# tsinghua-fib-lab/PIML

Measured on AMD Instinct MI355X. Metric: agent-pair force evals/sec + simulated steps/sec, 4096-agent GC scene, higher is better.
Workload: dtype f32

## Files before the change

piml_amd/csrc/encoder_bwd5.hip:

```cpp
#include "common.hpp"
#include "encoder.hpp"
#include "x3.hpp"

namespace piml {

typedef short f5_s16x4 __attribute__((ext_vector_type(4)));
typedef __attribute__((address_space(3))) f5_s16x4 f5_lds_s16x4;

constexpr int F5_THREADS = 512;
constexpr int F5_IMG = 3 * 128 * 64;
constexpr int F5_M = 0;
constexpr int F5_H = F5_M + 2 * F5_IMG;
constexpr int F5_TROW = 36;
constexpr int F5_TBYTES = 128 * F5_TROW * 4;
constexpr int F5_T = F5_H + 2 * F5_IMG;
constexpr int F5_XS = F5_T + 2 * F5_TBYTES;
constexpr int F5_MK = F5_XS + 3 * 1024;
constexpr int F5_W1 = F5_MK + 2 * 512;
constexpr int F5_GXP = F5_W1 + 4096;
#ifndef PIML_F5_PHASED
#define PIML_F5_PHASED 1
#endif
#ifndef PIML_F5_REQ_EARLY
#define PIML_F5_REQ_EARLY 0
#endif
#ifndef PIML_F5_GX_MFMA
#define PIML_F5_GX_MFMA 1
#endif
#ifndef PIML_F5_DW1_MFMA
#define PIML_F5_DW1_MFMA 0
#endif
static_assert(!PIML_F5_GX_MFMA || PIML_F5_PHASED, "the g_x products ride in the phased schedule");
static_assert(!PIML_F5_DW1_MFMA || PIML_F5_GX_MFMA, "the dW1 products need the zero region the g_x products freed");
constexpr int F5_GXP_BYTES = PIML_F5_GX_MFMA ? 4 * 32 * 16 * 4 : 4096;
constexpr int F5_TAB = F5_GXP + 2 * F5_GXP_BYTES;
constexpr int F5_KMAX = 16;
constexpr int F5_LDS_BYTES = F5_TAB + F5_KMAX * 2 * 16 * 4;
constexpr int F5_LDS_LAUNCH = F5_LDS_BYTES;
static_assert(F5_LDS_LAUNCH <= 160 * 1024, "fits the CU");
constexpr int F5_PART1 = EH * EH + 1024 + 2 * EH;

struct F5Args {
    EncArgs A;
    int nA[2];
    DecSlotSums D;
};

#ifndef PIML_F5_DEC_AT
#define PIML_F5_DEC_AT 1
#endif

template <int C>
__device__ __forceinline__ float f5_row_shl(float v) {
    return __int_as_float(__builtin_amdgcn_mov_dpp(__float_as_int(v), 0x100 + C, 0xf, 0xf, false));
}
template <int C>
__device__ __forceinline__ void f5_chains_add(float4& s, const float4 v) {
    if constexpr (C < 16) {
        slot_chains_add(s, make_float4(f5_row_shl<C>(v.x), f5_row_shl<C>(v.y), f5_row_shl<C>(v.z), f5_row_shl<C>(v.w)));
        f5_chains_add<C + 1>(s, v);
    }
}
__device__ __forceinline__ void f5_dec_sums(const DecSlotSums& D, int wg, int nwg, int t, int nthr) {
    const int total = D.nsets * D.lanes, per = (total + nwg - 1) / nwg;
    const int e1 = min(wg * per + per, total), half = nthr >> 4;
    for (int e = wg * per + (t >> 4); e < e1; e += 2 * half) {
        const bool two = e + half < e1;
        const int ea = e, eb = two ? e + half : e;
        const int sa = ea >= D.lanes ? 1 : 0, sb = eb >= D.lanes ? 1 : 0;
        const float4* const p[2] = {reinterpret_cast<const float4*>(sa ? D.parts[1] : D.parts[0]),
                                    reinterpret_cast<const float4*>(sb ? D.parts[1] : D.parts[0])};
        const int j[2] = {ea - sa * D.lanes, eb - sb * D.lanes};
        float4 s[2];
        slot_chains<2>(p, D.slots, D.lanes, j, t & 15, s);
        const float4 va = s[0], vb = s[1];
        f5_chains_add<1>(s[0], va);
        f5_chains_add<1>(s[1], vb);
        if ((t & 15) == 0) {
            slot_sum_store(reinterpret_cast<float4*>(sa ? D.grads[1] : D.grads[0]) + j[0], s[0], D.accumulate != 0);
            if (two) slot_sum_store(reinterpret_cast<float4*>(sb ? D.grads[1] : D.grads[0]) + j[1], s[1], D.accumulate != 0);
        }
    }
}

#ifdef PIML_F5_STAMPS
__device__ unsigned long long g_f5_stamps[256 * 8 * 16];
#define F5_STAMP(i)                                                        \
    do {                                                                   \
        __builtin_amdgcn_sched_barrier(0);                                 \
        {                                                                  \
            const unsigned long long t_ = __builtin_amdgcn_s_memtime();    \
            st[i] += t_ - tprev;                                           \
            tprev = t_;                                                    \
        }                                                                  \
        __builtin_amdgcn_sched_barrier(0);                                 \
    } while (0)
#else
#define F5_STAMP(i)
#endif

#define F5_BARRIER() asm volatile("s_waitcnt lgkmcnt(0)\n\ts_barrier" ::: "memory")

__device__ __forceinline__ float f5_relu(float x) { return __int_as_float(max(__float_as_int(x), 0)); }
__device__ __forceinline__ constexpr int f5_rho(int r) { return (r & 3) + 8 * (r >> 2); }

#ifndef PIML_F5_SKIP
#define PIML_F5_SKIP 0
#endif

#define F5_SLOT(MF, FILL)                        \
    do {                                         \
        MF;                                      \
        __builtin_amdgcn_sched_barrier(0);       \
        FILL;                                    \
        __builtin_amdgcn_sched_barrier(0);       \
    } while (0)

template <bool GX, int INC>
__global__ __launch_bounds__(F5_THREADS) void enc_bwd_sums2_kernel(F5Args F) {
    extern __shared__ __align__(16) unsigned char smem[];
    const int tid = threadIdx.x, lane = tid & 63;
    const int wv = __builtin_amdgcn_readfirstlane(tid >> 6);
    const int crew = wv >> 2, w = wv & 3;
    const int ctid = tid & 255;
    const int n = lane & 31, h = lane >> 5;
    int bx = (int)blockIdx.x, b = 0;
    if (bx >= F.nA[0]) { b = 1; bx -= F.nA[0]; }
    const piml_encoder_branch J = b ? F.A.br[1] : F.A.br[0];
    const int nwg = F.nA[b];
    const unsigned R = (unsigned)J.rows;
    const unsigned IN = __builtin_amdgcn_readfirstlane((unsigned)J.in_dim), K = __builtin_amdgcn_readfirstlane((unsigned)J.k);
    const unsigned kmagic = __builtin_amdgcn_readfirstlane((unsigned)((0x100000000ull + K - 1) / K));
    const int ntiles = (int)((R + 31) >> 5);
    const int nit = bx < ntiles ? (ntiles - bx + nwg - 1) / nwg : 0;
    float* P = J.partials + (size_t)bx * F5_PART1;
    constexpr int NS = INC == 6 ? 3 : 4;

    auto rsrc = [&](const void* base, unsigned bytes) {
        return __builtin_amdgcn_make_buffer_rsrc(const_cast<void*>(base), 0, (int)bytes, 0x00020000);
    };
    constexpr unsigned kOut = 0x80000000u;
    const __amdgpu_buffer_rsrc_t rs_gp = rsrc(J.g_pooled, (R / K) * EH * 4);
    const __amdgpu_buffer_rsrc_t rs_x = rsrc(J.x, R * IN * 4);
    const __amdgpu_buffer_rsrc_t rs_mk = rsrc(J.relu_mask, (unsigned)ntiles * 1024);
    const __amdgpu_buffer_rsrc_t rs_gx = rsrc(J.g_x, GX ? R * IN * 4 : 0u);
    auto ld1 = [&](const __amdgpu_buffer_rsrc_t& rs, unsigned voff, unsigned soff) {
        return (unsigned)__builtin_amdgcn_raw_buffer_load_b32(rs, (int)voff, (int)soff, 0);
    };

#ifdef PIML_F5_STAMPS
    unsigned long long st[16], tprev = __builtin_amdgcn_s_memtime();
#pragma unroll
    for (int i = 0; i < 16; ++i) st[i] = 0;
#endif

    {
        float4* z = reinterpret_cast<float4*>(smem + F5_T);
        constexpr int NZ = (F5_W1 - F5_T) / 16;
#pragma unroll
        for (int i = 0; i < (NZ + F5_THREADS - 1) / F5_THREADS; ++i)
            if (i * F5_THREADS + tid < NZ) z[i * F5_THREADS + tid] = make_float4(0.f, 0.f, 0.f, 0.f);
#pragma unroll
        for (int i = 0; i < 2 * F5_GXP_BYTES / 16 / F5_THREADS; ++i) reinterpret_cast<float4*>(smem + F5_GXP)[i * F5_THREADS + tid] = make_float4(0.f, 0.f, 0.f, 0.f);
        if ((unsigned)tid < K * 32u) {
            const unsigned rem = (unsigned)tid >> 5, hh = ((unsigned)tid >> 4) & 1u, r = (unsigned)tid & 15u;
            reinterpret_cast<unsigned*>(smem + F5_TAB)[tid] = ((rem + 4u * hh + (unsigned)f5_rho((int)r)) / K) * (EH * 4);
        }
        if (tid < 256 && PIML_F5_GX_MFMA) {
            reinterpret_cast<float4*>(smem + F5_W1)[tid] = make_float4(0.f, 0.f, 0.f, 0.f);
        } else if (tid < 256) {
            const float* W1r = J.packed + PACK_FWD + 32768;
            if (INC == 6) {
                const float* src = W1r + (tid >> 1) * 8 + 3 * (tid & 1);
                reinterpret_cast<float4*>(smem + F5_W1)[tid] = make_float4(src[0], src[1], src[2], 0.f);
            } else {
                reinterpret_cast<float4*>(smem + F5_W1)[tid] = reinterpret_cast<const float4*>(W1r)[tid];
            }
        }
    }

    if (crew == 0) {
        u32x4 wh[8], wm[8], wl[8];
        {
            const u32x4* imgB = reinterpret_cast<const u32x4*>(J.packed + PACK_F32 + 3 * X3_IMG) + lane;
#pragma unroll
            for (int kb = 0; kb < 8; ++kb) {
                const int fb = w * 8 + kb;
                wh[kb] = imgB[(fb * 2) * 64];
                wm[kb] = imgB[(fb * 2 + 1) * 64];
                wl[kb] = imgB[X3_HM / 4 + fb * 64];
            }
        }
        const float* W1rows = J.packed + PACK_FWD + 32768;
        float w1v[NS];
#pragma unroll
        for (int s = 0; s < NS; ++s) w1v[s] = W1rows[(32 * w + n) * 8 + 2 * s + h];
        const float b1v = J.b1[32 * w + n];

        const int fw = 32 * w + n;
        const int swz_w = (fw >> 1) & 7;
        const int mw_off = F5_M + fw * 64;
        int mr[2];
        {
            const int g16 = lane >> 4, q = (lane >> 2) & 3, pp = lane & 3, hh = g16 >> 1;
            const int chunk = 4 * (g16 & 1) + pp;
#pragma unroll
            for (int half2 = 0; half2 < 2; ++half2)
                mr[half2] = F5_M + (8 * half2 + 4 * hh + q) * 64 + ((chunk ^ (4 * half2 + 2 * hh + (q >> 1))) * 8);
        }
        const int bp = 16 * (w & 1) + (n & 3) + 4 * (n >> 3);
        const int mk_off = F5_MK + ((4 * h + 32 * ((n >> 2) & 1)) * 2 + (w >> 1)) * 4;
        const int t_off = F5_T + fw * (F5_TROW * 4) + (4 * h) * 4;
        const int h_off = F5_H + ((w * 2) * 3 * 64 + lane) * 16;
        const unsigned gbase = (unsigned)(32 * w + n) * 4u;

        float g2[16];
        unsigned m2 = 0, mkv = 0;
        float xa[NS];
        auto req_g = [&](int tile) {
            const unsigned t32 = __builtin_amdgcn_readfirstlane((unsigned)tile * 32u);
            const unsigned a0 = __builtin_amdgcn_readfirstlane(__umulhi(t32, kmagic)), rem = t32 - a0 * K;
            const bool live = tile < ntiles;
            const unsigned gb = live ? gbase + a0 * (EH * 4) : kOut;
            const uint4* tab = reinterpret_cast<const uint4*>(smem + F5_TAB + (rem * 32u + 16u * (unsigned)h) * 4u);
#pragma unroll
            for (int i = 0; i < 4; ++i) {
                const uint4 o = tab[i];
                g2[4 * i + 0] = __uint_as_float(ld1(rs_gp, gb + o.x, 0u));
                g2[4 * i + 1] = __uint_as_float(ld1(rs_gp, gb + o.y, 0u));
                g2[4 * i + 2] = __uint_as_float(ld1(rs_gp, gb + o.z, 0u));
                g2[4 * i + 3] = __uint_as_float(ld1(rs_gp, gb + o.w, 0u));
            }
            m2 = ld1(rs_mk, live ? (unsigned)tile * 1024u + (128u + 2u * (unsigned)lane + (unsigned)(w >> 1)) * 4u : kOut, 0u);
        };
        auto req_x = [&](int tile) {
            const unsigned row = (unsigned)tile * 32u + (unsigned)n;
            const bool valid = (tile < ntiles) & (row < R);
#pragma unroll
            for (int s = 0; s < NS; ++s) {
                const unsigned cx = 2u * s + h;
                xa[s] = __uint_as_float(ld1(rs_x, (valid & (cx < IN)) ? (row * IN + cx) * 4u : kOut, 0u));
            }
            mkv = ld1(rs_mk, tile < ntiles ? (unsigned)tile * 1024u + (unsigned)(ctid & 127) * 4u : kOut, 0u);
        };
        float g2n[16];
        unsigned m2n = 0, mkvn = 0;
        float xan[NS];
        uint4 tabv;
        auto req_step = [&](int i, int tile) {
            const unsigned t32 = __builtin_amdgcn_readfirstlane((unsigned)tile * 32u);
            const unsigned a0 = __builtin_amdgcn_readfirstlane(__umulhi(t32, kmagic)), rem = t32 - a0 * K;
            const bool live = tile < ntiles;
            const uint4* tab = reinterpret_cast<const uint4*>(smem + F5_TAB + (rem * 32u + 16u * (unsigned)h) * 4u);
            if (i == 0) { tabv = tab[0]; return; }
            if (i <= 4) {
                const unsigned gb = live ? gbase + a0 * (EH * 4) : kOut;
                const uint4 o = tabv;
                if (i < 4) tabv = tab[i];
                g2n[4 * i - 4] = __uint_as_float(ld1(rs_gp, gb + o.x, 0u));
                g2n[4 * i - 3] = __uint_as_float(ld1(rs_gp, gb + o.y, 0u));
                g2n[4 * i - 2] = __uint_as_float(ld1(rs_gp, gb + o.z, 0u));
                g2n[4 * i - 1] = __uint_as_float(ld1(rs_gp, gb + o.w, 0u));
                return;
            }
            m2n = ld1(rs_mk, live ? (unsigned)tile * 1024u + (128u + 2u * (unsigned)lane + (unsigned)(w >> 1)) * 4u : kOut, 0u);
            const unsigned row = (unsigned)tile * 32u + (unsigned)n;
            const bool valid = live & (row < R);
#pragma unroll
            for (int s = 0; s < NS; ++s) {
                const unsigned cx = 2u * s + h;
                xan[s] = __uint_as_float(ld1(rs_x, (valid & (cx < IN)) ? (row * IN + cx) * 4u : kOut, 0u));
            }
            mkvn = ld1(rs_mk, live ? (unsigned)tile * 1024u + (unsigned)(ctid & 127) * 4u : kOut, 0u);
        };
        auto req_take = [&]() {
#pragma unroll
            for (int r = 0; r < 16; ++r) g2[r] = g2n[r];
#pragma unroll
            for (int s = 0; s < NS; ++s) xa[s] = xan[s];
            m2 = m2n; mkv = mkvn;
        };
        float db1 = 0.f, db2 = 0.f;
        unsigned phi[4], pmid[4], plo[4];
        float sp_ra = 0.f, sp_rb = 0.f;
        auto split_a = [&](float a_, float b_, unsigned& hi) {
            hi = bf16_pair(a_, b_);
            sp_ra = a_ - __uint_as_float(hi << 16);
            sp_rb = b_ - __uint_as_float(hi & 0xffff0000u);
        };
        auto split_b = [&](unsigned& mid, unsigned& lo) {
            mid = bf16_pair(sp_ra, sp_rb);
            lo = bf16_pair(sp_ra - __uint_as_float(mid << 16), sp_rb - __uint_as_float(mid & 0xffff0000u));
        };
        auto g2_step = [&](int j, int pm) {
            const int s = j >> 3, q = j & 7;
            if (q < 2) {
                const unsigned m2w = m2 >> (16 * (w & 1));
#pragma unroll
                for (int r = 8 * s + 4 * q; r < 8 * s + 4 * q + 4; ++r) {
                    const int t = __builtin_amdgcn_sbfe(m2w, r, 1);
                    g2[r] = __uint_as_float(__float_as_uint(g2[r]) & (unsigned)t);
                    db2 += g2[r];
                }
            } else if (q < 6) {
                const int d = q - 2;
                split_a(g2[8 * s + 2 * d], g2[8 * s + 2 * d + 1], phi[d]);
                split_b(pmid[d], plo[d]);
            } else {
                const int g = 2 * s + (q - 6), d = 2 * (g & 1);
                unsigned char* dst = smem + mw_off + pm * F5_IMG + (((2 * g + h) ^ swz_w) * 8);
                *reinterpret_cast<uint2*>(dst) = make_uint2(phi[d], phi[d + 1]);
                *reinterpret_cast<uint2*>(dst + 8192) = make_uint2(pmid[d], pmid[d + 1]);
                *reinterpret_cast<uint2*>(dst + 16384) = make_uint2(plo[d], plo[d + 1]);
            }
        };
        f32x16 hacc;
        auto h1_mma = [&]() {
#pragma unroll
            for (int r = 0; r < 16; ++r) hacc[r] = b1v;
#pragma unroll
            for (int s = 0; s < NS; ++s) hacc = mfma32(xa[s], w1v[s], hacc);
        };
        auto h1_step = [&](int j, int pm) {
            const int s = j / 5, q = j % 5;
            if (q < 4) {
                split_a(f5_relu(hacc[8 * s + 2 * q]), f5_relu(hacc[8 * s + 2 * q + 1]), phi[q]);
                split_b(pmid[q], plo[q]);
            } else {
                u32x4* dst = reinterpret_cast<u32x4*>(smem + h_off + pm * F5_IMG + (s * 3 * 64) * 16);
                dst[0] = (u32x4){phi[0], phi[1], phi[2], phi[3]};
                dst[64] = (u32x4){pmid[0], pmid[1], pmid[2], pmid[3]};
                dst[128] = (u32x4){plo[0], plo[1], plo[2], plo[3]};
            }
        };
        auto stage = [&](int xslot, int pm) {
            if (w < NS) reinterpret_cast<float*>(smem + F5_XS + xslot * 1024)[n * 8 + 2 * w + h] = w == 0 ? xa[0] : (w == 1 ? xa[1] : (w == 2 ? xa[2] : xa[NS - 1]));
            if (ctid < 128) reinterpret_cast<unsigned*>(smem + F5_MK + pm * 512)[ctid] = mkv;
        };
        auto load_b = [&](u32x4 (&o)[3], int kb, int pm) {
#pragma unroll
            for (int p = 0; p < 3; ++p) {
                const f5_s16x4 lo4 = __builtin_amdgcn_ds_read_tr16_b64_v4i16((f5_lds_s16x4*)(smem + mr[0] + pm * F5_IMG + kb * 1024 + p * 8192));
                const f5_s16x4 hi4 = __builtin_amdgcn_ds_read_tr16_b64_v4i16((f5_lds_s16x4*)(smem + mr[1] + pm * F5_IMG + kb * 1024 + p * 8192));
                const uint2 x = __builtin_bit_cast(uint2, lo4), y = __builtin_bit_cast(uint2, hi4);
                o[p] = (u32x4){x.x, x.y, y.x, y.y};
            }
        };

        F5_BARRIER();
        req_g(bx);
        req_x(bx);
#pragma unroll
        for (int j = 0; j < 16; ++j) g2_step(j, 0);
        h1_mma();
#pragma unroll
        for (int j = 0; j < 10; ++j) h1_step(j, 0);
        stage(0, 0);
        req_g(bx + nwg);
        req_x(bx + nwg);
        F5_STAMP(15);
        F5_BARRIER();

        for (int it = 0; it < nit; ++it) {
            const int par = it & 1, tile = bx + it * nwg;
            F5_STAMP(0);
            f32x16 acc;
            u32x4 opa[2][3], ahi[8];
            unsigned mkw[16];
            const unsigned* mk1 = reinterpret_cast<const unsigned*>(smem + mk_off + par * 512);
            auto fill_a = [&](int sl) {
                if (sl < 40 && sl % 5 == 0) {
                    const int kb = sl / 5 + 1;
                    if (kb < 8) load_b(opa[kb & 1], kb, par);
                    return;
                }
                if (sl == 38 || sl == 39) return;
                const int f = sl < 40 ? sl - sl / 5 - 1 : sl - 10;
                if (PIML_F5_PHASED) {
                    if (PIML_F5_REQ_EARLY && f >= 2 && f < 14 && !(f & 1) && !(PIML_F5_SKIP & 128)) req_step(f / 2 - 1, tile + 2 * nwg);
                    if (f >= 30 && f < 34) {
#pragma unroll
                        for (int i = 4 * (f - 30); i < 4 * (f - 30) + 4; ++i) mkw[i] = mk1[2 * f5_rho(i)];
                    }
                    return;
                }
                if (f < 16) { if (!(PIML_F5_SKIP & 4)) g2_step(f, par ^ 1); }
                else if (f < 20) {
#pragma unroll
                    for (int i = 4 * (f - 16); i < 4 * (f - 16) + 4; ++i) mkw[i] = mk1[2 * f5_rho(i)];
                }
                else if (f == 20) { if (!(PIML_F5_SKIP & 8)) h1_mma(); }
                else if (f >= 23 && f < 33) { if (!(PIML_F5_SKIP & 8)) h1_step(f - 23, par ^ 1); }
                else if (f == 33) stage((it + 1) % 3, par ^ 1);
                else if (f == 34) { if (!(PIML_F5_SKIP & 128)) req_g(tile + 2 * nwg); }
                else if (f == 35) { if (!(PIML_F5_SKIP & 128)) req_x(tile + 2 * nwg); }
            };
            load_b(opa[0], 0, par);
            const f32x16 zero16 = {0.f, 0.f, 0.f, 0.f, 0.f, 0.f, 0.f, 0.f, 0.f, 0.f, 0.f, 0.f, 0.f, 0.f, 0.f, 0.f};
#pragma unroll
            for (int kb = 0; kb < 8; ++kb) {
                const u32x4 (&o)[3] = opa[kb & 1];
                ahi[kb] = o[0];
#define F5_MA(X) do { if (!(PIML_F5_SKIP & 64)) { X; } else if (kb == 0) acc = zero16; } while (0)
                F5_SLOT(F5_MA(acc = mfma_bf(o[2], wh[kb], kb == 0 ? zero16 : acc)), fill_a(kb * 5 + 0));
                F5_SLOT(F5_MA(acc = mfma_bf(o[1], wm[kb], acc)), fill_a(kb * 5 + 1));
                F5_SLOT(F5_MA(acc = mfma_bf(o[0], wl[kb], acc)), fill_a(kb * 5 + 2));
                F5_SLOT(F5_MA(acc = mfma_bf(o[1], wh[kb], acc)), fill_a(kb * 5 + 3));
                F5_SLOT(F5_MA(acc = mfma_bf(o[0], wm[kb], acc)), fill_a(kb * 5 + 4));
            }
#ifdef PIML_F5_ACC2
            f32x16 acc2 = zero16;
#pragma unroll
            for (int kb = 0; kb < 8; ++kb) F5_SLOT(if (kb & 1) acc2 = mfma_bf(ahi[kb], wh[kb], acc2); else acc = mfma_bf(ahi[kb], wh[kb], acc), fill_a(40 + kb));
#pragma unroll
            for (int r = 0; r < 16; ++r) acc[r] += acc2[r];
#else
#pragma unroll
            for (int kb = 0; kb < 8; ++kb) F5_SLOT(F5_MA(acc = mfma_bf(ahi[kb], wh[kb], acc)), fill_a(40 + kb));
#endif
            F5_STAMP(1);
            if (!(PIML_F5_SKIP & 16))
#pragma unroll
            for (int r = 0; r < 16; ++r) {
                const int t = __builtin_amdgcn_sbfe(mkw[r], bp, 1);
                acc[r] = __uint_as_float(__float_as_uint(acc[r]) & (unsigned)t);
                db1 += acc[r];
            }
            if (!(PIML_F5_SKIP & 16)) {
                float4* dst = reinterpret_cast<float4*>(smem + t_off + par * F5_TBYTES);
#pragma unroll
                for (int g = 0; g < 4; ++g) dst[2 * g] = make_float4(acc[4 * g], acc[4 * g + 1], acc[4 * g + 2], acc[4 * g + 3]);
            }
            F5_STAMP(2);
            if (PIML_F5_PHASED) {
                if (!(PIML_F5_SKIP & 8)) h1_mma();
                if (!(PIML_F5_SKIP & 4)) {
#pragma unroll
                    for (int j = 0; j < 16; ++j) g2_step(j, par ^ 1);
                }
                F5_STAMP(6);
                if (!(PIML_F5_SKIP & 8)) {
#pragma unroll
                    for (int j = 0; j < 10; ++j) h1_step(j, par ^ 1);
                }
                F5_STAMP(7);
                stage((it + 1) % 3, par ^ 1);
                if (!(PIML_F5_SKIP & 128)) {
                    if (PIML_F5_REQ_EARLY) req_take();
                    else { req_g(tile + 2 * nwg); req_x(tile + 2 * nwg); }
                }
                F5_STAMP(5);
            }
            F5_BARRIER();
        }
        F5_STAMP(3);
        if (PIML_F5_DEC_AT == 1 && F.D.nsets > 0) {
            f5_dec_sums(F.D, (int)blockIdx.x, (int)gridDim.x, ctid, 256);
            F5_STAMP(12);
        }
        F5_BARRIER();
        F5_BARRIER();
        db1 += __shfl_xor(db1, 32, 64);
        db2 += __shfl_xor(db2, 32, 64);
        if (h == 0) {
            P[EH * EH + 1024 + 32 * w + n] = db2;
            P[EH * EH + 1024 + EH + 32 * w + n] = db1;
        }
        for (unsigned cc = IN * 128 + ctid; cc < 1024; cc += 256) P[EH * EH + cc] = 0.f;
        F5_STAMP(11);
    } else {
        f32x16 c[4], sm[4];
#pragma unroll
        for (int jb = 0; jb < 4; ++jb)
#pragma unroll
            for (int r = 0; r < 16; ++r) { c[jb][r] = 0.f; sm[jb][r] = 0.f; }
        float w1acc[INC];
#pragma unroll
        for (int cc = 0; cc < INC; ++cc) w1acc[cc] = 0.f;
        float w1g[8];
        {
            const float* W1r = J.packed + PACK_FWD + 32768;
#pragma unroll
            for (int j = 0; j < 8; ++j) w1g[j] = (lane & 15) < 8 ? W1r[(32 * w + 4 * j + (lane >> 4)) * 8 + (lane & 15)] : 0.f;
        }
        const int fw = 32 * w + n;
        const int swz_w = (fw >> 1) & 7;
        const int mw_off = F5_M + fw * 64;
        const int t_row = F5_T + fw * (F5_TROW * 4) + (4 * h) * 4;
        const int t_col = F5_T + (32 * w) * (F5_TROW * 4) + n * 4;
        const int w1_off = F5_W1 + (32 * w) * 32 + h * 16;
        const int xs_off = F5_XS + (4 * h) * 32;

        auto load_g2 = [&](u32x4 (&g)[3], int s_, int pm) {
#pragma unroll
            for (int p = 0; p < 3; ++p) {
                const uint2 x = *reinterpret_cast<const uint2*>(smem + mw_off + pm * F5_IMG + p * 8192 + (((4 * s_ + h) ^ swz_w) * 8));
                const uint2 y = *reinterpret_cast<const uint2*>(smem + mw_off + pm * F5_IMG + p * 8192 + (((4 * s_ + 2 + h) ^ swz_w) * 8));
                g[p] = (u32x4){x.x, x.y, y.x, y.y};
            }
        };
        auto load_h = [&](u32x4 (&o)[3], int u_, int pm) {
            const int s_ = u_ >> 2, jb_ = u_ & 3;
            const u32x4* hr = reinterpret_cast<const u32x4*>(smem + F5_H + pm * F5_IMG) + lane;
#pragma unroll
            for (int p = 0; p < 3; ++p) o[p] = hr[((jb_ * 2 + s_) * 3 + p) * 64];
        };
        auto gx_store = [&](int tile, int pm) {
            const unsigned grow = (unsigned)tile * 32u + (unsigned)(ctid >> 3), cs = (unsigned)ctid & 7u;
            float v;
            if (PIML_F5_GX_MFMA) {
                const float* gp = reinterpret_cast<const float*>(smem + F5_GXP + pm * F5_GXP_BYTES) + (ctid >> 3) * 16 + (ctid & 7);
                v = ((gp[0] + gp[512]) + gp[1024]) + gp[1536];
            } else {
                const float* gp = reinterpret_cast<const float*>(smem + F5_GXP + pm * F5_GXP_BYTES) + ctid;
                v = ((gp[0] + gp[256]) + gp[512]) + gp[768];
            }
            const unsigned cx = (INC == 6 && !PIML_F5_GX_MFMA) ? 3u * (cs >> 2) + (cs & 3u) : cs;
            const bool cok = (INC == 6 && !PIML_F5_GX_MFMA) ? (cs & 3u) != 3u : cx < IN;
            const unsigned off = (grow * IN + cx) * 4u;
            __builtin_amdgcn_raw_buffer_store_b32(__float_as_uint(v), rs_gx, (int)(((tile >= 0) & (tile < ntiles) & (grow < R) & cok) ? off : kOut), 0, 0);
        };
#ifndef PIML_F5_GXD
#define PIML_F5_GXD 1
#endif
        constexpr int GXR = PIML_F5_GXD + 1;
        float gx[4];
        float tv[GXR][2];
        float4 tw[GXR][2];
        auto gx_load = [&](int k, int pm) {
#pragma unroll
            for (int e = 0; e < 2; ++e) {
                if (PIML_F5_SKIP & 512) tv[k % GXR][e] = (float)k; else
                tv[k % GXR][e] = *reinterpret_cast<const float*>(smem + t_col + pm * F5_TBYTES + (2 * k + e) * (F5_TROW * 4));
                if (PIML_F5_SKIP & 256) tw[k % GXR][e] = make_float4(1.f, 2.f, 3.f, (float)k); else
                tw[k % GXR][e] = *reinterpret_cast<const float4*>(smem + w1_off + (2 * k + e) * 32);
            }
        };
        auto gx_fma = [&](int k) {
#pragma unroll
            for (int e = 0; e < 2; ++e) {
                const float v = tv[k % GXR][e];
                const float4 wv = tw[k % GXR][e];
                gx[0] = __fmaf_rn(wv.x, v, gx[0]); gx[1] = __fmaf_rn(wv.y, v, gx[1]);
                gx[2] = __fmaf_rn(wv.z, v, gx[2]);
                if (INC == 8) gx[3] = __fmaf_rn(wv.w, v, gx[3]);
            }
        };
        float g1[16];
        float4 xv[2][4];
        auto g1_load = [&](int half_, int pm) {
            const float4* src = reinterpret_cast<const float4*>(smem + t_row + pm * F5_TBYTES);
#pragma unroll
            for (int g = 2 * half_; g < 2 * half_ + 2; ++g) {
                const float4 v = src[2 * g];
                g1[4 * g] = v.x; g1[4 * g + 1] = v.y; g1[4 * g + 2] = v.z; g1[4 * g + 3] = v.w;
            }
        };
        auto x_load = [&](int k, int xslot) {
            const float4* xr = reinterpret_cast<const float4*>(smem + xs_off + xslot * 1024);
#pragma unroll
            for (int e = 0; e < 2; ++e) {
                xv[k & 1][2 * e] = xr[2 * f5_rho(2 * k + e)];
                if (INC == 8) xv[k & 1][2 * e + 1] = xr[2 * f5_rho(2 * k + e) + 1];
                else {
                    const float2 t2 = *reinterpret_cast<const float2*>(&xr[2 * f5_rho(2 * k + e) + 1]);
                    xv[k & 1][2 * e + 1] = make_float4(t2.x, t2.y, 0.f, 0.f);
                }
            }
        };
        auto x_fma = [&](int k) {
#pragma unroll
            for (int e = 0; e < 2; ++e) {
                const float4 xa4 = xv[k & 1][2 * e], xb4 = xv[k & 1][2 * e + 1];
                const float g = g1[2 * k + e];
                w1acc[0] = __fmaf_rn(g, xa4.x, w1acc[0]); w1acc[1] = __fmaf_rn(g, xa4.y, w1acc[1]);
                w1acc[2] = __fmaf_rn(g, xa4.z, w1acc[2]); w1acc[3] = __fmaf_rn(g, xa4.w, w1acc[3]);
                w1acc[4] = __fmaf_rn(g, xb4.x, w1acc[4]); w1acc[5] = __fmaf_rn(g, xb4.y, w1acc[5]);
                if (INC == 8) { w1acc[INC - 2] = __fmaf_rn(g, xb4.z, w1acc[INC - 2]); w1acc[INC - 1] = __fmaf_rn(g, xb4.w, w1acc[INC - 1]); }
            }
        };
        f32x4 gd[2];
        float ga[8][2];
        const int ga_off = F5_T + (32 * w + (lane >> 4)) * (F5_TROW * 4) + (lane & 15) * 4;
        auto gm_load = [&](int j, int pm) {
#pragma unroll
            for (int r = 0; r < 2; ++r) ga[j][r] = *reinterpret_cast<const float*>(smem + ga_off + pm * F5_TBYTES + j * (4 * F5_TROW * 4) + r * 64);
        };
        f32x4 dw1m[2] = {(f32x4){0.f, 0.f, 0.f, 0.f}, (f32x4){0.f, 0.f, 0.f, 0.f}};
        float da[8][2], dbv[8];
        const int da_off = F5_T + (32 * w + (lane & 15)) * (F5_TROW * 4) + (lane >> 4) * 4;
        const int db_off = (lane & 15) < 8 ? F5_XS + (lane >> 4) * 32 + (lane & 15) * 4 : F5_W1 + (lane >> 4) * 32;
        auto dwm_step = [&](int f, int pm, int xslot) {
            if (f < 2) {
#pragma unroll
                for (int j = 4 * f; j < 4 * f + 4; ++j) {
#pragma unroll
                    for (int c2 = 0; c2 < 2; ++c2) da[j][c2] = *reinterpret_cast<const float*>(smem + da_off + pm * F5_TBYTES + c2 * (16 * F5_TROW * 4) + j * 16);
                    dbv[j] = *reinterpret_cast<const float*>(smem + db_off + xslot * 1024 + j * 128);
                }
            } else {
                const int j = f - 2;
#pragma unroll
                for (int c2 = 0; c2 < 2; ++c2) dw1m[c2] = __builtin_amdgcn_mfma_f32_16x16x4f32(da[j][c2], dbv[j], dw1m[c2], 0, 0, 0);
            }
        };
        auto gxm_step = [&](int f, int pm) {
            if (!GX) return;
            if (f == 0) {
                gd[0] = gd[1] = (f32x4){0.f, 0.f, 0.f, 0.f};
#pragma unroll
                for (int j = 0; j < 8; ++j) gm_load(j, pm);
            } else if (f <= 8) {
                const int j = f - 1;
#pragma unroll
                for (int r = 0; r < 2; ++r) gd[r] = __builtin_amdgcn_mfma_f32_16x16x4f32(ga[j][r], w1g[j], gd[r], 0, 0, 0);
            } else if (f == 9) {
                float* dst = reinterpret_cast<float*>(smem + F5_GXP + (pm ^ 1) * F5_GXP_BYTES) + (w * 32 + 4 * (lane >> 4)) * 16 + (lane & 15);
#pragma unroll
                for (int r = 0; r < 2; ++r)
#pragma unroll
                    for (int i = 0; i < 4; ++i) dst[(16 * r + i) * 16] = gd[r][i];
            }
        };
        auto lag_step_m = [&](int f, int pm, int xslot) {
            if (PIML_F5_DW1_MFMA) return;
            if (f == 0) { g1_load(0, pm); g1_load(1, pm); x_load(0, xslot); }
            else if (f == 1) { x_load(1, xslot); x_fma(0); }
            else if (f < 9) { if (f < 8) x_load(f, xslot); x_fma(f - 1); }
        };
        auto lag_step_v = [&](int f, int pm, int xslot) {
            if (f == 0) {
                gx[0] = gx[1] = gx[2] = gx[3] = 0.f;
                if (GX && !(PIML_F5_SKIP & 2)) {
#pragma unroll
                    for (int k = 0; k < PIML_F5_GXD; ++k) gx_load(k, pm);
                }
            } else if (f <= 16) {
                if (GX && !(PIML_F5_SKIP & 2)) { if (f - 1 + PIML_F5_GXD < 16) gx_load(f - 1 + PIML_F5_GXD, pm); gx_fma(f - 1); }
                if (f == 15) g1_load(0, pm);
                if (f == 16) { g1_load(1, pm); x_load(0, xslot); }
            } else if (f == 17) {
                if (GX) reinterpret_cast<float4*>(smem + F5_GXP + (pm ^ 1) * F5_GXP_BYTES)[(w * 32 + n) * 2 + h] = make_float4(gx[0], gx[1], gx[2], gx[3]);
                x_load(1, xslot); x_fma(0);
            } else if (f < 25) {
                if (f < 24) x_load(f - 16, xslot);
                x_fma(f - 17);
            }
        };
        auto lag_step = [&](int f, int pm, int xslot) {
            if (PIML_F5_GX_MFMA) lag_step_m(f, pm, xslot); else lag_step_v(f, pm, xslot);
        };

#ifdef PIML_F5_PRIO_B
        __builtin_amdgcn_s_setprio(PIML_F5_PRIO_B);
#endif
        F5_BARRIER();
        F5_STAMP(15);
        F5_BARRIER();
        for (int it = 0; it < nit; ++it) {
            const int par = it & 1, tile = bx + it * nwg;
            F5_STAMP(0);
            u32x4 g2f[3], opb[2][3];
            const int lpm = par ^ 1, xslot = (it + 2) % 3;
            auto fill_b = [&](int sl) {
                if (sl % 6 == 0) {
                    const int u_ = sl / 6 + 1;
                    if (u_ < 8) load_h(opb[u_ & 1], u_, par);
                    return;
                }
                if (sl == 23) { load_g2(g2f, 1, par); return; }
                const int f = sl - sl / 6 - 1 - (sl > 23);
                if (PIML_F5_PHASED) {
                    if (PIML_F5_GX_MFMA && !(PIML_F5_SKIP & 2)) {
                        if (f == 1) gxm_step(0, lpm);
                        else if (f >= 6 && f < 14) gxm_step(f - 5, lpm);
                        else if (f == 22) gxm_step(9, lpm);
                    }
                    if (PIML_F5_DW1_MFMA && !(PIML_F5_SKIP & 1)) {
                        if (f == 2 || f == 3) dwm_step(f - 2, lpm, xslot);
                        else if (f >= 14 && f < 22) dwm_step(f - 12, lpm, xslot);
                    }
                    return;
                }
                if (PIML_F5_SKIP & 1) return;
                if (f == 0) { if (GX) gx_store(tile - 2 * nwg, par ^ 1); }
                else if (f < 28) lag_step(f - 1, lpm, xslot);
            };
            if (PIML_F5_PHASED && !(PIML_F5_SKIP & 1)) {
                if (GX) gx_store(tile - 2 * nwg, par ^ 1);
#pragma unroll
                for (int f = 0; f < 17; ++f) lag_step(f, lpm, xslot);
                F5_STAMP(6);
#pragma unroll
                for (int f = 17; f < 27; ++f) lag_step(f, lpm, xslot);
                F5_STAMP(5);
            }
#ifdef PIML_F5_PRIO_PROD
            __builtin_amdgcn_s_setprio(PIML_F5_PRIO_PROD);
#endif
            load_g2(g2f, 0, par);
            load_h(opb[0], 0, par);
#pragma unroll
            for (int u = 0; u < 8; ++u) {
                const int jb = u & 3;
                const u32x4 (&o)[3] = opb[u & 1];
#define F5_MB(X) do { if (!(PIML_F5_SKIP & 32)) { X; } } while (0)
                F5_SLOT(F5_MB(sm[jb] = mfma_bf(g2f[2], o[0], sm[jb])), fill_b(u * 6 + 0));
                F5_SLOT(F5_MB(sm[jb] = mfma_bf(g2f[1], o[1], sm[jb])), fill_b(u * 6 + 1));
                F5_SLOT(F5_MB(sm[jb] = mfma_bf(g2f[0], o[2], sm[jb])), fill_b(u * 6 + 2));
                F5_SLOT(F5_MB(sm[jb] = mfma_bf(g2f[1], o[0], sm[jb])), fill_b(u * 6 + 3));
                F5_SLOT(F5_MB(sm[jb] = mfma_bf(g2f[0], o[1], sm[jb])), fill_b(u * 6 + 4));
                F5_SLOT(F5_MB(c[jb] = mfma_bf(g2f[0], o[0], c[jb])), fill_b(u * 6 + 5));
            }
#ifdef PIML_F5_PRIO_PROD
            __builtin_amdgcn_s_setprio(0);
#endif
            F5_STAMP(1);
            F5_BARRIER();
        }
        F5_STAMP(3);
        {
            const int it = nit, par = it & 1, tile = bx + it * nwg;
            if (GX) gx_store(tile - 2 * nwg, par ^ 1);
#pragma unroll
            for (int f = 0; f < 27; ++f) lag_step(f, par ^ 1, (it + 2) % 3);
            if (PIML_F5_GX_MFMA) {
#pragma unroll
                for (int f = 0; f < 10; ++f) gxm_step(f, par ^ 1);
            }
            if (PIML_F5_DW1_MFMA) {
#pragma unroll
                for (int f = 0; f < 10; ++f) dwm_step(f, par ^ 1, (it + 2) % 3);
            }
            F5_BARRIER();
            if (GX) gx_store(tile - nwg, par);
            F5_BARRIER();
        }
        F5_STAMP(4);
#pragma unroll
        for (int jb = 0; jb < 4; ++jb)
#pragma unroll
            for (int r = 0; r < 16; ++r) P[(size_t)(32 * w + f5_rho(r) + 4 * h) * EH + 32 * jb + n] = c[jb][r] + sm[jb][r];
        if (PIML_F5_DW1_MFMA) {
            if ((unsigned)(lane & 15) < IN) {
#pragma unroll
                for (int c2 = 0; c2 < 2; ++c2)
#pragma unroll
                    for (int i = 0; i < 4; ++i) P[EH * EH + (size_t)(32 * w + 16 * c2 + 4 * (lane >> 4) + i) * IN + (lane & 15)] = dw1m[c2][i];
            }
        } else {
#pragma unroll
            for (int cc = 0; cc < INC; ++cc) w1acc[cc] += __shfl_xor(w1acc[cc], 32, 64);
            if (h == 0) {
                float* o = P + EH * EH + (size_t)(32 * w + n) * IN;
#pragma unroll
                for (int cc = 0; cc < INC; ++cc)
                    if ((unsigned)cc < IN) o[cc] = w1acc[cc];
            }
        }
        F5_STAMP(11);
    }
    if (PIML_F5_DEC_AT == 0 && F.D.nsets > 0) {
        f5_dec_sums(F.D, (int)blockIdx.x, (int)gridDim.x, tid, F5_THREADS);
        F5_STAMP(12);
    }
#ifdef PIML_F5_STAMPS
    if (lane == 0)
        for (int i = 0; i < 16; ++i) g_f5_stamps[(blockIdx.x * 8 + wv) * 16 + i] = st[i];
#endif
}

#ifdef PIML_F5_STAMPS
extern "C" __attribute__((visibility("default"))) int piml_f5_stamps(unsigned long long* out) {
    return (int)hipMemcpyFromSymbol(out, HIP_SYMBOL(g_f5_stamps), sizeof(unsigned long long) * 256 * 8 * 16);
}
#endif

int enc_f5_set_attributes() {
    auto set = [&](const void* f) { return (int)hipFuncSetAttribute(f, hipFuncAttributeMaxDynamicSharedMemorySize, F5_LDS_LAUNCH); };
    if (int e = set(reinterpret_cast<const void*>(enc_bwd_sums2_kernel<false, 6>))) return e;
    if (int e = set(reinterpret_cast<const void*>(enc_bwd_sums2_kernel<true, 6>))) return e;
    if (int e = set(reinterpret_cast<const void*>(enc_bwd_sums2_kernel<false, 8>))) return e;
    return set(reinterpret_cast<const void*>(enc_bwd_sums2_kernel<true, 8>));
}

bool enc_f5_launch(const EncArgs& A, const int* nA, hipStream_t s, const DecSlotSums* D) {
    F5Args F;
    F.A = A;
    F.nA[0] = nA[0]; F.nA[1] = A.nbr > 1 ? nA[1] : 0;
    F.D = D ? *D : DecSlotSums{};
    bool in6 = true;
    for (int i = 0; i < A.nbr; ++i) {
        if (A.br[i].k > F5_KMAX) return false;
        in6 = in6 && A.br[i].in_dim == 6;
    }
    const bool gx = A.br[0].g_x != nullptr;
    const dim3 g((unsigned)(F.nA[0] + F.nA[1])), blk(F5_THREADS);
    if (in6) {
        if (gx) hipLaunchKernelGGL((enc_bwd_sums2_kernel<true, 6>), g, blk, F5_LDS_LAUNCH, s, F);
        else hipLaunchKernelGGL((enc_bwd_sums2_kernel<false, 6>), g, blk, F5_LDS_LAUNCH, s, F);
    } else {
        if (gx) hipLaunchKernelGGL((enc_bwd_sums2_kernel<true, 8>), g, blk, F5_LDS_LAUNCH, s, F);
        else hipLaunchKernelGGL((enc_bwd_sums2_kernel<false, 8>), g, blk, F5_LDS_LAUNCH, s, F);
    }
    return true;
}

}
```

Measured before the change: 229.0 billion.

## Overlap encoder-backward prologue and tail with decoder slot-sum prefetch

Moves the LDS zeroing and table setup onto the consumer crew so the producer crew can issue its first gradient, mask and x loads before the first barrier, and defers weight-register loads until after those requests. It restructures the tail: the last iteration skips its phased prep and barrier, the decoder slot-sum reduction prefetches its first batch of partials before the barrier, and the final gx store moves to the producer crew, which removes two barriers. The slot-chain reduction becomes an explicit 8-deep unrolled load-and-add loop. It also adds optional memtime/realtime marks for profiling. The cost is more live registers for the prefetched partials and a more fragile barrier count between the crews.

After: 231.9 billion (median of 6 runs). 1.01x the previous value.

```diff
diff --git a/piml_amd/csrc/encoder_bwd5.hip b/piml_amd/csrc/encoder_bwd5.hip
--- a/piml_amd/csrc/encoder_bwd5.hip
+++ b/piml_amd/csrc/encoder_bwd5.hip
@@ -61,24 +61,64 @@
         f5_chains_add<C + 1>(s, v);
     }
 }
-__device__ __forceinline__ void f5_dec_sums(const DecSlotSums& D, int wg, int nwg, int t, int nthr) {
+struct F5DecCols {
+    const float4* p[2];
+    float4* g[2];
+    int j[2];
+    bool two;
+};
+__device__ __forceinline__ F5DecCols f5_dec_cols(const DecSlotSums& D, int e, int e1, int half) {
+    F5DecCols C;
+    C.two = e + half < e1;
+    const int ea = e, eb = C.two ? e + half : e;
+    const int sa = ea >= D.lanes ? 1 : 0, sb = eb >= D.lanes ? 1 : 0;
+    C.p[0] = reinterpret_cast<const float4*>(sa ? D.parts[1] : D.parts[0]);
+    C.p[1] = reinterpret_cast<const float4*>(sb ? D.parts[1] : D.parts[0]);
+    C.g[0] = reinterpret_cast<float4*>(sa ? D.grads[1] : D.grads[0]);
+    C.g[1] = reinterpret_cast<float4*>(sb ? D.grads[1] : D.grads[0]);
+    C.j[0] = ea - sa * D.lanes;
+    C.j[1] = eb - sb * D.lanes;
+    return C;
+}
+__device__ __forceinline__ void f5_dec_load(const DecSlotSums& D, const F5DecCols& C, int q0, int c, float4 (&v)[2][8]) {
+#pragma unroll
+    for (int m = 0; m < 2; ++m)
+#pragma unroll
+        for (int u = 0; u < 8; ++u) {
+            const int q = q0 + 16 * u;
+            v[m][u] = C.p[m][(size_t)(q < D.slots ? q : c) * D.lanes + C.j[m]];
+        }
+}
+__device__ __forceinline__ void f5_dec_first(const DecSlotSums& D, int wg, int nwg, int t, int nthr, float4 (&v)[2][8]) {
     const int total = D.nsets * D.lanes, per = (total + nwg - 1) / nwg;
-    const int e1 = min(wg * per + per, total), half = nthr >> 4;
+    const int e1 = min(wg * per + per, total), e = wg * per + (t >> 4);
+    if (e < e1) f5_dec_load(D, f5_dec_cols(D, e, e1, nthr >> 4), t & 15, t & 15, v);
+}
+__device__ __forceinline__ void f5_dec_sums(const DecSlotSums& D, int wg, int nwg, int t, int nthr, float4 (&v)[2][8]) {
+    const int total = D.nsets * D.lanes, per = (total + nwg - 1) / nwg;
+    const int e1 = min(wg * per + per, total), half = nthr >> 4, c = t & 15;
+    bool pre = true;
     for (int e = wg * per + (t >> 4); e < e1; e += 2 * half) {
-        const bool two = e + half < e1;
-        const int ea = e, eb = two ? e + half : e;
-        const int sa = ea >= D.lanes ? 1 : 0, sb = eb >= D.lanes ? 1 : 0;
-        const float4* const p[2] = {reinterpret_cast<const float4*>(sa ? D.parts[1] : D.parts[0]),
-                                    reinterpret_cast<const float4*>(sb ? D.parts[1] : D.parts[0])};
-        const int j[2] = {ea - sa * D.lanes, eb - sb * D.lanes};
+        const F5DecCols C = f5_dec_cols(D, e, e1, half);
         float4 s[2];
-        slot_chains<2>(p, D.slots, D.lanes, j, t & 15, s);
+        s[0] = s[1] = make_float4(0.f, 0.f, 0.f, 0.f);
+        for (int q0 = c; q0 < D.slots; q0 += 16 * 8) {
+            if (!pre) f5_dec_load(D, C, q0, c, v);
+            pre = false;
+#pragma unroll
+            for (int m = 0; m < 2; ++m)
+#pragma unroll
+                for (int u = 0; u < 8; ++u) {
+                    const bool ok = q0 + 16 * u < D.slots;
+                    s[m].x += ok ? v[m][u].x : 0.f; s[m].y += ok ? v[m][u].y : 0.f; s[m].z += ok ? v[m][u].z : 0.f; s[m].w += ok ? v[m][u].w : 0.f;
+                }
+        }
         const float4 va = s[0], vb = s[1];
         f5_chains_add<1>(s[0], va);
         f5_chains_add<1>(s[1], vb);
-        if ((t & 15) == 0) {
-            slot_sum_store(reinterpret_cast<float4*>(sa ? D.grads[1] : D.grads[0]) + j[0], s[0], D.accumulate != 0);
-            if (two) slot_sum_store(reinterpret_cast<float4*>(sb ? D.grads[1] : D.grads[0]) + j[1], s[1], D.accumulate != 0);
+        if (c == 0) {
+            slot_sum_store(C.g[0] + C.j[0], s[0], D.accumulate != 0);
+            if (C.two) slot_sum_store(C.g[1] + C.j[1], s[1], D.accumulate != 0);
         }
     }
 }
@@ -95,8 +135,17 @@
         }                                                                  \
         __builtin_amdgcn_sched_barrier(0);                                 \
     } while (0)
+__device__ unsigned long long g_f5_marks[256 * 8 * 8];
+#define F5_MARK(i)                                                         \
+    do {                                                                   \
+        __builtin_amdgcn_sched_barrier(0);                                 \
+        mk_[2 * (i)] = __builtin_amdgcn_s_memtime();                       \
+        mk_[2 * (i) + 1] = __builtin_amdgcn_s_memrealtime();               \
+        __builtin_amdgcn_sched_barrier(0);                                 \
+    } while (0)
 #else
 #define F5_STAMP(i)
+#define F5_MARK(i)
 #endif
 
 #define F5_BARRIER() asm volatile("s_waitcnt lgkmcnt(0)\n\ts_barrier" ::: "memory")
@@ -149,53 +198,58 @@
     };
 
 #ifdef PIML_F5_STAMPS
-    unsigned long long st[16], tprev = __builtin_amdgcn_s_memtime();
+    unsigned long long st[16], mk_[8], tprev = __builtin_amdgcn_s_memtime();
 #pragma unroll
     for (int i = 0; i < 16; ++i) st[i] = 0;
-#endif
-
-    {
-        float4* z = reinterpret_cast<float4*>(smem + F5_T);
-        constexpr int NZ = (F5_W1 - F5_T) / 16;
-#pragma unroll
-        for (int i = 0; i < (NZ + F5_THREADS - 1) / F5_THREADS; ++i)
-            if (i * F5_THREADS + tid < NZ) z[i * F5_THREADS + tid] = make_float4(0.f, 0.f, 0.f, 0.f);
-#pragma unroll
-        for (int i = 0; i < 2 * F5_GXP_BYTES / 16 / F5_THREADS; ++i) reinterpret_cast<float4*>(smem + F5_GXP)[i * F5_THREADS + tid] = make_float4(0.f, 0.f, 0.f, 0.f);
-        if ((unsigned)tid < K * 32u) {
-            const unsigned rem = (unsigned)tid >> 5, hh = ((unsigned)tid >> 4) & 1u, r = (unsigned)tid & 15u;
-            reinterpret_cast<unsigned*>(smem + F5_TAB)[tid] = ((rem + 4u * hh + (unsigned)f5_rho((int)r)) / K) * (EH * 4);
-        }
-        if (tid < 256 && PIML_F5_GX_MFMA) {
-            reinterpret_cast<float4*>(smem + F5_W1)[tid] = make_float4(0.f, 0.f, 0.f, 0.f);
-        } else if (tid < 256) {
+    F5_MARK(0);
+#endif
+
+    if (crew == 1) {
+        float4* z = reinterpret_cast<float4*>(smem + F5_T + F5_TBYTES);
+        constexpr int NZ = F5_TBYTES / 16;
+#pragma unroll
+        for (int i = 0; i < (NZ + 255) / 256; ++i)
+            if (i * 256 + ctid < NZ) z[i * 256 + ctid] = make_float4(0.f, 0.f, 0.f, 0.f);
+        if (ctid < 64) reinterpret_cast<float4*>(smem + F5_XS + 2 * 1024)[ctid] = make_float4(0.f, 0.f, 0.f, 0.f);
+#pragma unroll
+        for (int e0 = 0; e0 < F5_KMAX * 32; e0 += 256) {
+            const unsigned e = (unsigned)(e0 + ctid);
+            if (e < K * 32u) {
+                const unsigned rem = e >> 5, hh = (e >> 4) & 1u, r = e & 15u;
+                reinterpret_cast<unsigned*>(smem + F5_TAB)[e] = ((rem + 4u * hh + (unsigned)f5_rho((int)r)) / K) * (EH * 4);
+            }
+        }
+        if (PIML_F5_GX_MFMA) {
+            reinterpret_cast<float4*>(smem + F5_W1)[ctid] = make_float4(0.f, 0.f, 0.f, 0.f);
+        } else {
             const float* W1r = J.packed + PACK_FWD + 32768;
             if (INC == 6) {
-                const float* src = W1r + (tid >> 1) * 8 + 3 * (tid & 1);
-                reinterpret_cast<float4*>(smem + F5_W1)[tid] = make_float4(src[0], src[1], src[2], 0.f);
+                const float* src = W1r + (ctid >> 1) * 8 + 3 * (ctid & 1);
+                reinterpret_cast<float4*>(smem + F5_W1)[ctid] = make_float4(src[0], src[1], src[2], 0.f);
             } else {
-                reinterpret_cast<float4*>(smem + F5_W1)[tid] = reinterpret_cast<const float4*>(W1r)[tid];
+                reinterpret_cast<float4*>(smem + F5_W1)[ctid] = reinterpret_cast<const float4*>(W1r)[ctid];
             }
         }
     }
 
+    auto gx_store = [&](int tile, int pm) {
+        const unsigned grow = (unsigned)tile * 32u + (unsigned)(ctid >> 3), cs = (unsigned)ctid & 7u;
+        float v;
+        if (PIML_F5_GX_MFMA) {
+            const float* gp = reinterpret_cast<const float*>(smem + F5_GXP + pm * F5_GXP_BYTES) + (ctid >> 3) * 16 + (ctid & 7);
+            v = ((gp[0] + gp[512]) + gp[1024]) + gp[1536];
+        } else {
+            const float* gp = reinterpret_cast<const float*>(smem + F5_GXP + pm * F5_GXP_BYTES) + ctid;
+            v = ((gp[0] + gp[256]) + gp[512]) + gp[768];
+        }
+        const unsigned cx = (INC == 6 && !PIML_F5_GX_MFMA) ? 3u * (cs >> 2) + (cs & 3u) : cs;
+        const bool cok = (INC == 6 && !PIML_F5_GX_MFMA) ? (cs & 3u) != 3u : cx < IN;
+        const unsigned off = (grow * IN + cx) * 4u;
+        __builtin_amdgcn_raw_buffer_store_b32(__float_as_uint(v), rs_gx, (int)(((tile >= 0) & (tile < ntiles) & (grow < R) & cok) ? off : kOut), 0, 0);
+    };
+
     if (crew == 0) {
-        u32x4 wh[8], wm[8], wl[8];
-        {
-            const u32x4* imgB = reinterpret_cast<const u32x4*>(J.packed + PACK_F32 + 3 * X3_IMG) + lane;
-#pragma unroll
-            for (int kb = 0; kb < 8; ++kb) {
-                const int fb = w * 8 + kb;
-                wh[kb] = imgB[(fb * 2) * 64];
-                wm[kb] = imgB[(fb * 2 + 1) * 64];
-                wl[kb] = imgB[X3_HM / 4 + fb * 64];
-            }
-        }
-        const float* W1rows = J.packed + PACK_FWD + 32768;
-        float w1v[NS];
-#pragma unroll
-        for (int s = 0; s < NS; ++s) w1v[s] = W1rows[(32 * w + n) * 8 + 2 * s + h];
-        const float b1v = J.b1[32 * w + n];
+        float w1v[NS], b1v;
 
         const int fw = 32 * w + n;
         const int swz_w = (fw >> 1) & 7;
@@ -347,9 +401,36 @@
             }
         };
 
+        {
+            const unsigned t32 = __builtin_amdgcn_readfirstlane((unsigned)bx * 32u);
+            const unsigned a0 = __builtin_amdgcn_readfirstlane(__umulhi(t32, kmagic)), rem = t32 - a0 * K;
+            const unsigned gb = bx < ntiles ? gbase + a0 * (EH * 4) : kOut;
+#pragma unroll
+            for (int r = 0; r < 16; ++r) {
+                const unsigned m = rem + 4u * (unsigned)h + (unsigned)f5_rho(r);
+                g2[r] = __uint_as_float(ld1(rs_gp, gb + (K == 1u ? m : __umulhi(m, kmagic)) * (EH * 4), 0u));
+            }
+            m2 = ld1(rs_mk, bx < ntiles ? (unsigned)bx * 1024u + (128u + 2u * (unsigned)lane + (unsigned)(w >> 1)) * 4u : kOut, 0u);
+        }
+        req_x(bx);
+        {
+            const float* W1rows = J.packed + PACK_FWD + 32768;
+#pragma unroll
+            for (int s = 0; s < NS; ++s) w1v[s] = W1rows[(32 * w + n) * 8 + 2 * s + h];
+            b1v = J.b1[32 * w + n];
+        }
+        u32x4 wh[8], wm[8], wl[8];
+        {
+            const u32x4* imgB = reinterpret_cast<const u32x4*>(J.packed + PACK_F32 + 3 * X3_IMG) + lane;
+#pragma unroll
+            for (int kb = 0; kb < 8; ++kb) {
+                const int fb = w * 8 + kb;
+                wh[kb] = imgB[(fb * 2) * 64];
+                wm[kb] = imgB[(fb * 2 + 1) * 64];
+                wl[kb] = imgB[X3_HM / 4 + fb * 64];
+            }
+        }
         F5_BARRIER();
-        req_g(bx);
-        req_x(bx);
 #pragma unroll
         for (int j = 0; j < 16; ++j) g2_step(j, 0);
         h1_mma();
@@ -364,6 +445,7 @@
         for (int it = 0; it < nit; ++it) {
             const int par = it & 1, tile = bx + it * nwg;
             F5_STAMP(0);
+            if (it == 0) F5_MARK(1);
             f32x16 acc;
             u32x4 opa[2][3], ahi[8];
             unsigned mkw[16];
@@ -432,7 +514,7 @@
                 for (int g = 0; g < 4; ++g) dst[2 * g] = make_float4(acc[4 * g], acc[4 * g + 1], acc[4 * g + 2], acc[4 * g + 3]);
             }
             F5_STAMP(2);
-            if (PIML_F5_PHASED) {
+            if (PIML_F5_PHASED && it + 1 < nit) {
                 if (!(PIML_F5_SKIP & 8)) h1_mma();
                 if (!(PIML_F5_SKIP & 4)) {
 #pragma unroll
@@ -451,15 +533,20 @@
                 }
                 F5_STAMP(5);
             }
-            F5_BARRIER();
+            if (it + 1 < nit) F5_BARRIER();
         }
         F5_STAMP(3);
-        if (PIML_F5_DEC_AT == 1 && F.D.nsets > 0) {
-            f5_dec_sums(F.D, (int)blockIdx.x, (int)gridDim.x, ctid, 256);
+        const bool dec = PIML_F5_DEC_AT == 1 && F.D.nsets > 0;
+        float4 dv[2][8];
+        if (dec) f5_dec_first(F.D, (int)blockIdx.x, (int)gridDim.x, ctid, 256, dv);
+        if (nit > 0) F5_BARRIER();
+        F5_MARK(2);
+        if (dec) {
+            f5_dec_sums(F.D, (int)blockIdx.x, (int)gridDim.x, ctid, 256, dv);
             F5_STAMP(12);
         }
         F5_BARRIER();
-        F5_BARRIER();
+        if (GX) gx_store(bx + (nit - 1) * nwg, nit & 1);
         db1 += __shfl_xor(db1, 32, 64);
         db2 += __shfl_xor(db2, 32, 64);
         if (h == 0) {
@@ -504,21 +591,6 @@
             const u32x4* hr = reinterpret_cast<const u32x4*>(smem + F5_H + pm * F5_IMG) + lane;
 #pragma unroll
             for (int p = 0; p < 3; ++p) o[p] = hr[((jb_ * 2 + s_) * 3 + p) * 64];
-        };
-        auto gx_store = [&](int tile, int pm) {
-            const unsigned grow = (unsigned)tile * 32u + (unsigned)(ctid >> 3), cs = (unsigned)ctid & 7u;
-            float v;
-            if (PIML_F5_GX_MFMA) {
-                const float* gp = reinterpret_cast<const float*>(smem + F5_GXP + pm * F5_GXP_BYTES) + (ctid >> 3) * 16 + (ctid & 7);
-                v = ((gp[0] + gp[512]) + gp[1024]) + gp[1536];
-            } else {
-                const float* gp = reinterpret_cast<const float*>(smem + F5_GXP + pm * F5_GXP_BYTES) + ctid;
-                v = ((gp[0] + gp[256]) + gp[512]) + gp[768];
-            }
-            const unsigned cx = (INC == 6 && !PIML_F5_GX_MFMA) ? 3u * (cs >> 2) + (cs & 3u) : cs;
-            const bool cok = (INC == 6 && !PIML_F5_GX_MFMA) ? (cs & 3u) != 3u : cx < IN;
-            const unsigned off = (grow * IN + cx) * 4u;
-            __builtin_amdgcn_raw_buffer_store_b32(__float_as_uint(v), rs_gx, (int)(((tile >= 0) & (tile < ntiles) & (grow < R) & cok) ? off : kOut), 0, 0);
         };
 #ifndef PIML_F5_GXD
 #define PIML_F5_GXD 1
@@ -660,6 +732,7 @@
         for (int it = 0; it < nit; ++it) {
             const int par = it & 1, tile = bx + it * nwg;
             F5_STAMP(0);
+            if (it == 0) F5_MARK(1);
             u32x4 g2f[3], opb[2][3];
             const int lpm = par ^ 1, xslot = (it + 2) % 3;
             auto fill_b = [&](int sl) {
@@ -719,6 +792,7 @@
             F5_BARRIER();
         }
         F5_STAMP(3);
+        F5_MARK(2);
         {
             const int it = nit, par = it & 1, tile = bx + it * nwg;
             if (GX) gx_store(tile - 2 * nwg, par ^ 1);
@@ -732,9 +806,6 @@
 #pragma unroll
                 for (int f = 0; f < 10; ++f) dwm_step(f, par ^ 1, (it + 2) % 3);
             }
-            F5_BARRIER();
-            if (GX) gx_store(tile - nwg, par);
-            F5_BARRIER();
         }
         F5_STAMP(4);
 #pragma unroll
@@ -758,21 +829,30 @@
                     if ((unsigned)cc < IN) o[cc] = w1acc[cc];
             }
         }
+        F5_BARRIER();
         F5_STAMP(11);
     }
     if (PIML_F5_DEC_AT == 0 && F.D.nsets > 0) {
-        f5_dec_sums(F.D, (int)blockIdx.x, (int)gridDim.x, tid, F5_THREADS);
+        float4 dv[2][8];
+        f5_dec_first(F.D, (int)blockIdx.x, (int)gridDim.x, tid, F5_THREADS, dv);
+        f5_dec_sums(F.D, (int)blockIdx.x, (int)gridDim.x, tid, F5_THREADS, dv);
         F5_STAMP(12);
     }
 #ifdef PIML_F5_STAMPS
-    if (lane == 0)
+    F5_MARK(3);
+    if (lane == 0 && blockIdx.x < 256) {
         for (int i = 0; i < 16; ++i) g_f5_stamps[(blockIdx.x * 8 + wv) * 16 + i] = st[i];
+        for (int i = 0; i < 8; ++i) g_f5_marks[(blockIdx.x * 8 + wv) * 8 + i] = mk_[i];
+    }
 #endif
 }
 
 #ifdef PIML_F5_STAMPS
 extern "C" __attribute__((visibility("default"))) int piml_f5_stamps(unsigned long long* out) {
     return (int)hipMemcpyFromSymbol(out, HIP_SYMBOL(g_f5_stamps), sizeof(unsigned long long) * 256 * 8 * 16);
+}
+extern "C" __attribute__((visibility("default"))) int piml_f5_marks(unsigned long long* out) {
+    return (int)hipMemcpyFromSymbol(out, HIP_SYMBOL(g_f5_marks), sizeof(unsigned long long) * 256 * 8 * 8);
 }
 #endif
 
```
